# BGU-CS-VIL/DPMMSubClusters.jl

Hardware: AMD Instinct MI355X
Metric: Gibbs iterations/sec, N=10M D=64 NIW (higher is better)
Workload: dtype f32

## Files before the change

### dpmmsubclusters.jl_amd/binding.py

```python
import ctypes
import os
import subprocess

import numpy as np

_HERE = os.path.dirname(os.path.abspath(__file__))
PRIOR_NIW, PRIOR_MULT = 0, 1
MAX_CLUSTERS = 1024

_c_i64p = ctypes.POINTER(ctypes.c_int64)
_c_f32p = ctypes.POINTER(ctypes.c_float)
_c_f64p = ctypes.POINTER(ctypes.c_double)

ABI = [
    ("dpmm_abi_version", ctypes.c_int, []),
    ("dpmm_create", ctypes.c_int, [ctypes.POINTER(ctypes.c_void_p), ctypes.c_int, ctypes.c_int, ctypes.c_int64, ctypes.c_int64, ctypes.c_int, ctypes.c_uint64]),
    ("dpmm_destroy", ctypes.c_int, [ctypes.c_void_p]),
    ("dpmm_last_error", ctypes.c_char_p, [ctypes.c_void_p]),
    ("dpmm_upload_points", ctypes.c_int, [ctypes.c_void_p, _c_f32p, ctypes.c_int64]),
    ("dpmm_upload_points_device", ctypes.c_int, [ctypes.c_void_p, ctypes.c_void_p, ctypes.c_int64]),
    ("dpmm_upload_points_npy", ctypes.c_int, [ctypes.c_void_p, ctypes.c_void_p, ctypes.c_int, ctypes.c_int64, ctypes.c_int]),
    ("dpmm_upload_points_csc", ctypes.c_int, [ctypes.c_void_p, _c_i64p, _c_i64p, _c_f32p, ctypes.c_int]),
    ("dpmm_init_labels", ctypes.c_int, [ctypes.c_void_p, ctypes.c_int, ctypes.c_uint32]),
    ("dpmm_set_labels", ctypes.c_int, [ctypes.c_void_p, _c_i64p, _c_i64p]),
# ... 154 lines not shown
]
SAMPLE_MAX_TRIALS_SPARSE = 4096
SAMPLE_MAX_TRIALS_DENSE = 1 << 24
OPT_SCORE_TABLE_MB = 32
SCORE_MAX_TOP = 16
ABI_MISSING = [
    ("dpmm_score_missing_counts", ctypes.c_int, [ctypes.c_void_p, _c_i64p]),
    ("dpmm_impute_points", ctypes.c_int, [ctypes.c_void_p, _c_f32p, ctypes.c_int64]),
    ("dpmm_impute_points_device", ctypes.c_int, [ctypes.c_void_p, ctypes.c_void_p, ctypes.c_int64]),
]
OPT_SCORE_MISSING = 33
SCORE_MAX_MISSING = 16
_IMPUTE_DRAW_TAIL = [ctypes.c_int64, ctypes.c_int64, ctypes.c_void_p, ctypes.c_uint64, ctypes.c_int64, ctypes.c_int64, ctypes.c_int64]
ABI_IMPUTE = [
    ("dpmm_impute_draw_points", ctypes.c_int, [ctypes.c_void_p, _c_f32p] + _IMPUTE_DRAW_TAIL),
    ("dpmm_impute_draw_points_device", ctypes.c_int, [ctypes.c_void_p, ctypes.c_void_p] + _IMPUTE_DRAW_TAIL),
]
IMPUTE_MAX_DRAWS = 1 << 26

HOST_ALLREDUCE_FN = ctypes.CFUNCTYPE(ctypes.c_int, ctypes.c_void_p, ctypes.c_void_p, ctypes.c_int64, ctypes.c_int)

MASTER_NSCALARS = 8
OPT_SCREEN_MARGIN, OPT_TAIL_SCREEN, OPT_PRESCREEN, OPT_ORDERED_SWEEP, OPT_MULT_FORCE_F32, OPT_STATS_ITEMS, OPT_STATS_GROUPS, OPT_TRACE_SLOW, OPT_LOGLIK_REF_CONST, OPT_WAVE_PRIO, OPT_MULT_NO_U8, OPT_SWEEP_GRID, OPT_SWEEP_QUEUE_ROUNDS, OPT_BALL_SCREEN, OPT_KERNEL_TIMING, OPT_STATS_DERIVE, OPT_NOISE_AHEAD, OPT_REF_BRACKET, OPT_SORT_TILE, OPT_ONE_COLLECTIVE, OPT_BF16_SCREENS, OPT_COMM_TIMEOUT_MS, OPT_DIRECTION_SCREEN, _OPT_RESERVED_24, OPT_MULT_DRAWS_AHEAD, OPT_B3_SUBLABELS, OPT_LEAN_TILES, OPT_MASTER_POLL, OPT_CHAIN_FUSION, OPT_LEAN_DIRECTION, OPT_PAIR_BALL = range(1, 32)


class DpmmError(RuntimeError):
    def __init__(self, code, msg):
        super().__init__(f"libdpmmhip error {code}: {msg}")
        self.code = code


def lib_path():
    return os.path.join(_HERE, "lib", "libdpmmhip.so")


def locked_make(args, lock_dir):
    import fcntl
    os.makedirs(lock_dir, exist_ok=True)
    with open(os.path.join(lock_dir, ".build.lock"), "w") as lk:
        fcntl.flock(lk, fcntl.LOCK_EX)
        try:
            subprocess.check_call(args)
        finally:
            fcntl.flock(lk, fcntl.LOCK_UN)


# ... 772 lines not shown
```

### dpmmsubclusters.jl_amd/csrc/dpmm_api.cpp

```cpp
#include "../../include/dpmm_hip.h"
#include "../../include/dpmm_hip_master.h"
#include "../../include/dpmm_hip_debug.h"
#include "../../include/dpmm_hip_tensor.h"
#include "../../include/dpmm_hip_csc.h"
#include "../../include/dpmm_hip_score.h"
#include "../../include/dpmm_hip_rank.h"
#include "../../include/dpmm_hip_overlap.h"
#include "../../include/dpmm_hip_trace.h"
#include "../../include/dpmm_hip_missing.h"
#include "../../include/dpmm_hip_impute.h"
#include "../../include/dpmm_hip_sample.h"
#include "../../include/dpmm_hip_project.h"

#include <hip/hip_runtime.h>
#include <dlfcn.h>

#include <algorithm>
#include <atomic>
#include <condition_variable>
#include <mutex>
#include <thread>
#include <chrono>
#include <cmath>
#include <cstdio>
// ... 216 lines not shown
    float opt_margin = 50.f;
    int opt_prio = 1;
    int opt_queue_rounds = -1;
    int opt_ball = 1;
    DevBuf<uint32_t> d_sp_frag;
    DevBuf<uint32_t> d_refb_big;
    bool have_refb_big = false;
    DevBuf<uint32_t> d_brk_flag;
    DevBuf<float> d_brk_aref;
    DevBuf<float> d_sp_cons;
    PinBuf<uint32_t> h_need;
    int opt_direction = -1;
    bool sp_ready = false, sp_regime = false;
    unsigned sp_count = 0;
    bool sp_last = false;
    int sp_K = -1;
    int sp_cooldown = 0;
    int opt_b3 = 1;
    bool have_b3 = false;
    int opt_chain = 0x7fffffff & ~(8 | 32);
    int opt_pair_ball = 1;
    bool have_pb = false;
    int opt_lean_dir = 1;
    int opt_master_poll = 1;
    int opt_lean = 1;
    DevBuf<uint32_t> d_hard;
    int hard_flip = 0;
    int perm_nbins = 0;
    PinBuf<uint32_t> h_hard;
    int lean_off = 0;
    bool lean_ran = false;
    int lean_backoff = 15;
    int opt_bf16scr = 1;
    int opt_bracket = 1;
    int opt_timing = 0;
    int opt_tail = 1, opt_prescreen = -1, opt_ordered = 1, opt_force_f32 = 0, opt_trace = 0, opt_ref_const = 0;
    int64_t opt_stats_items = 0;
    int opt_stats_groups = 0;
    void *comm = nullptr;
    int rank = 0, world = 1;
    dpmm_host_allreduce_fn host_fn = nullptr;
    void *host_user = nullptr;
    PinBuf<char> h_red;
    hipEvent_t ev_comm[4] = {nullptr, nullptr, nullptr, nullptr};
    bool have_comm_ev[2] = {false, false};
    int64_t comm_bytes[2] = {0, 0};
// ... 1682 lines not shown
        c->apairs_inflight = false; c->apairs_valid = true;
        c->apairs_req.clear();
    }
    const bool fused_pairs_launched = napairs > 0 && fuse_pairs;
    const bool need_event = !poll || (napairs > 0 && !fuse_pairs);
    if (need_event) HIPCHK(c, hipEventRecord(c->ev_master, c->stream));
    if (napairs > 0 && !fuse_pairs) {
        HIPCHK(c, hipStreamWaitEvent(c->stream2, c->ev_master, 0));
        HIPCHK(c, launch_niw_master_pairs(c->ma, c->d_apairs, napairs, c->d_pairs, c->h_apairs, c->stream2));
        HIPCHK(c, hipEventRecord(c->ev_pairs, c->stream2));
        c->apairs_index.clear();
        for (int p = 0; p < napairs; ++p) c->apairs_index[((uint32_t)c->apairs_req[2 * p] << 16) | (uint32_t)c->apairs_req[2 * p + 1]] = p;
        c->apairs_dirty.assign((size_t)c->master_slots, 0);
        c->apairs_inflight = true; c->apairs_valid = true;
        c->apairs_req.clear();
    }
    if (draw_epoch) {
        const int32_t *hs = c->d_dslots;
        const bool have_normals = normals_by_post || noise_ready(c, draw_epoch, K, c->draw_cur ^ 1);
        if (int rc = noise_join(c)) return rc;
        NiwMasterArgs ma = c->ma;
        ma.mu_draw = c->d_mu_draw[c->draw_cur ^ 1];
        HIPCHK(c, launch_niw_master_draw(ma, hs, K, draw_epoch, c->d_Y[c->draw_cur ^ 1], c->d_ld_sigma[c->draw_cur ^ 1], nullptr, nullptr,
                                         nullptr, nullptr, nullptr, nullptr, c->NB, nullptr, 1 | (have_normals ? 4 : 0), c->stream));
        c->noise_valid = false;
        c->spec_inflight = false; c->spec_valid = true; c->spec_epoch = draw_epoch;
        c->spec_slots.assign(slots, slots + K);
    }
    if (int rc = flush_undo(c)) return rc;
    if (poll) { if (int rc = wait_master_records(c, sm, 3 * (int64_t)K, c->h_apairs, fused_pairs_launched ? napairs : 0)) return rc; }
    else HIPCHK(c, sync_event(c, c->ev_master));
    if (master_marks_left(sm, K)) {
        ++c->dbg_early_wait;
        const auto t0 = std::chrono::steady_clock::now();
        while (master_marks_left(sm, K)) {
            if (std::chrono::steady_clock::now() - t0 > std::chrono::seconds(5)) return fail(c, DPMM_EHIP, "posterior records missing 5 s after the event wait returned");
            HIPCHK(c, sync_stream(c, c->stream));
        }
    }
    c->handover_inflight = false;
    *bad = reinterpret_cast<const uint8_t *>(c->h_out.get());
    *small = sm;
    return DPMM_OK;
}

int dpmm_suffstats_device(dpmm_ctx *c, const int64_t *idx, int n_idx) {
    if (!c) return DPMM_EINVAL;
// ... 40 lines not shown
    if (int rc = noise_flush(c)) return rc;
    if (int rc = ensure_capacity(c, K)) return rc;
    if (int rc = master_capacity(c, 0, K)) return rc;
    if (c->handover_inflight) HIPCHK(c, sync_stream(c, c->stream));
    c->handover_inflight = true;
    float *hlr = reinterpret_cast<float *>(c->h_draw.get()), *hw = hlr + 2 * K;
    memcpy(hlr, lr, sizeof(float) * 2 * K);
    memcpy(hw, w, sizeof(float) * K);
    c->have_tail = c->opt_tail && c->D >= 4 && c->D % 4 == 0 && K > 1;
    const bool ahead = c->spec_valid && c->spec_epoch == epoch && (int)c->spec_slots.size() == K &&
                       memcmp(c->spec_slots.data(), slot_of_cluster, sizeof(int32_t) * K) == 0;
    if (int rc = spec_join(c)) return rc;
    c->spec_valid = false;
    if (int rc = noise_join(c)) return rc;
    if (!ahead) if (int rc = device_list(c, c->d_dslots, c->dslots_shadow, slot_of_cluster, (size_t)K)) return rc;
    const int32_t *hs = c->d_dslots;
    c->draw_cur ^= 1;
    NiwMasterArgs ma = c->ma;
    ma.mu_draw = c->d_mu_draw[c->draw_cur];
    const bool normals = !ahead && noise_ready(c, epoch, K, c->draw_cur);
    c->predictive = false;
    const bool roles = (c->opt_chain & 2) != 0, b3_in_pack = roles && want_b3_images(c), pb_in_pack = b3_in_pack && want_pair_ball(c, K);
    HIPCHK(c, launch_niw_master_draw(ma, hs, K, epoch, c->d_Y[c->draw_cur], c->d_ld_sigma[c->draw_cur], hlr, hw, c->d_Rp, c->d_mup, c->d_cst,
                                     c->have_tail ? c->d_tail : nullptr, c->NB, c->d_work, (ahead ? 2 : (normals ? 7 : 3)) | (roles ? 8 : 0) | (b3_in_pack ? 16 : 0) | (pb_in_pack ? 32 : 0), c->stream));
    if (int rc = direction_tables(c, K, b3_in_pack, pb_in_pack)) return rc;
    c->noise_pending = c->opt_noise_ahead < 0 ? (c->D >= 128 || c->n < 4000000) : c->opt_noise_ahead != 0; c->noise_pend_epoch = epoch + 1; c->noise_pend_nmat = 3 * std::min(K + 4, c->master_K);
    if ((c->opt_chain & 16) && niw_master_can_fuse_pairs(c->ma)) c->noise_pending = false;
    c->work_zeroed = true;
    c->have_screen_prep = false;
    c->K = K;
    c->have_params = true;
    c->predictive = false;
    c->draws_on_device = true;
    return DPMM_OK;
}

int dpmm_niw_master_pairs_ahead(dpmm_ctx *c, const int32_t *slots_i, const int32_t *slots_j, int n) {
    if (!c || n < 0 || (n > 0 && (!slots_i || !slots_j))) return DPMM_EINVAL;
    if (!c->master) return fail(c, DPMM_ESTATE, "dpmm_niw_master_setup first");
    c->apairs_req.clear();
    for (int i = 0; i < n; ++i) {
        if (slots_i[i] < 0 || slots_i[i] >= DPMM_MAX_CLUSTERS || slots_j[i] < 0 || slots_j[i] >= DPMM_MAX_CLUSTERS) { c->apairs_req.clear(); return fail(c, DPMM_EINVAL, "slot out of range"); }
        c->apairs_req.push_back(slots_i[i]); c->apairs_req.push_back(slots_j[i]);
    }
    return DPMM_OK;
}

// ... 499 lines not shown
        case DPMM_OPT_PRESCREEN: c->opt_prescreen = value < 0 ? -1 : (value != 0); return DPMM_OK;
        case DPMM_OPT_ORDERED_SWEEP: c->opt_ordered = value != 0; return DPMM_OK;
        case DPMM_OPT_MULT_FORCE_F32:
            if (c->have_points) return fail(c, DPMM_ESTATE, "DPMM_OPT_MULT_FORCE_F32 must be set before the points are uploaded");
            c->opt_force_f32 = value != 0; return DPMM_OK;
        case DPMM_OPT_STATS_ITEMS:
            if (c->Kcap > 0) return fail(c, DPMM_ESTATE, "DPMM_OPT_STATS_ITEMS must be set before the first parameters / K");
            if (value >= 1) c->chunk_dense = c->chunk = (int)std::max<int64_t>((c->prior == DPMM_PRIOR_NIW && c->D <= 64) ? 32 : 256, ((c->n + (int64_t)value - 1) / (int64_t)value + 3) / 4 * 4);
            if (c->x_sparse) return set_points_chunk(c, true);
            return DPMM_OK;
        case DPMM_OPT_STATS_GROUPS: c->opt_stats_groups = value > 0 ? (int)value : 0; return DPMM_OK;
        case DPMM_OPT_TRACE_SLOW: c->opt_trace = value != 0; return DPMM_OK;
        case DPMM_OPT_LOGLIK_REF_CONST: c->opt_ref_const = value != 0; return DPMM_OK;
        case DPMM_OPT_WAVE_PRIO: c->opt_prio = value != 0; return DPMM_OK;
        case DPMM_OPT_MULT_DRAWS_AHEAD: c->opt_mult_draws_ahead = value != 0; c->mspec_valid = false; return DPMM_OK;
        case DPMM_OPT_SWEEP_QUEUE_ROUNDS: c->opt_queue_rounds = value < 0 ? -1 : (int)value; return DPMM_OK;
        case DPMM_OPT_BALL_SCREEN: c->opt_ball = value != 0; return DPMM_OK;
        case DPMM_OPT_STATS_DERIVE: c->opt_derive = value != 0; c->cache_force = true; return DPMM_OK;
        case DPMM_OPT_NOISE_AHEAD: c->opt_noise_ahead = value < 0 ? -1 : (value != 0); return DPMM_OK;
        case DPMM_OPT_REF_BRACKET: c->opt_bracket = value != 0; return DPMM_OK;
        case DPMM_OPT_COMM_TIMEOUT_MS: c->comm_timeout_ms = value > 0 ? (int)std::min(value, 2.0e9) : 0; return DPMM_OK;
        case DPMM_OPT_BF16_SCREENS: c->opt_bf16scr = value != 0; return DPMM_OK;
        case DPMM_OPT_MASTER_POLL: c->opt_master_poll = value != 0; return DPMM_OK;
        case DPMM_OPT_PAIR_BALL: c->opt_pair_ball = value != 0; if (!c->opt_pair_ball) c->have_pb = false; return DPMM_OK;
        case DPMM_OPT_LEAN_DIRECTION: c->opt_lean_dir = value != 0; c->lean_off = 0; c->lean_backoff = 15; c->lean_ran = false; return DPMM_OK;
        case DPMM_OPT_CHAIN_FUSION: c->opt_chain = value < 0 ? (0x7fffffff & ~(8 | 32)) : (int)value; return DPMM_OK;
        case DPMM_OPT_LEAN_TILES: c->opt_lean = value != 0; c->lean_off = 0; c->lean_backoff = 15; c->lean_ran = false; return DPMM_OK;
        case DPMM_OPT_B3_SUBLABELS: c->opt_b3 = value != 0; if (!c->opt_b3) c->have_b3 = false; return DPMM_OK;
        case DPMM_OPT_DIRECTION_SCREEN:
            c->opt_direction = value < 0 ? -1 : (value != 0);
            if (c->opt_direction == 0) { c->sp_ready = false; c->sp_regime = false; }
            return DPMM_OK;
        case DPMM_OPT_ONE_COLLECTIVE: c->opt_one_collective = value < 0 ? -1 : (value != 0); return DPMM_OK;
        case DPMM_OPT_SORT_TILE: {
            const int t = (int)value;
            if (t != SORT_TILE && t != SORT_TILE_SMALL) return fail(c, DPMM_EINVAL, "DPMM_OPT_SORT_TILE: 512 or 2048");
            if (t < c->sort_tile_min) {
                if (c->n > 16000000) return fail(c, DPMM_ELIMIT, "DPMM_OPT_SORT_TILE: 512-point tiles are limited to shards of 16e6 points");
                HIPCHK(c, hipSetDevice(c->device));
                HIPCHK(c, sync_stream(c, c->stream));
                const int nt = (int)((c->n + t - 1) / t);
                const size_t nbmax = 2 * DPMM_MAX_CLUSTERS;
                DevBuf<int32_t> th, tc, tsp;
                if (th.alloc(sizeof(int32_t) * nbmax * (size_t)std::max(1, nt)) != hipSuccess || tc.alloc(sizeof(int32_t) * nbmax * (size_t)std::max(1, nt)) != hipSuccess ||
                    tsp.alloc(sizeof(int32_t) * (size_t)STEP_SPEC_MAX_BINS * (size_t)std::max(1, nt)) != hipSuccess)
                    return fail(c, DPMM_EHIP, "DPMM_OPT_SORT_TILE: out of device memory for the 512-point tile tables");
// ... 1416 lines not shown
```

### dpmmsubclusters.jl_amd/csrc/niw_master.hip

```cpp
#include <algorithm>
#include "dpmm_device.h"
#include "dpmm_kernels.h"
#include "niw_b3.h"

namespace dpmm {

enum : uint32_t { STREAM_M_NORMAL = 32, STREAM_M_CHI = 33, STREAM_M_XI = 34 };
typedef double f64x4m __attribute__((ext_vector_type(4)));
constexpr int NS = DPMM_MASTER_NSCALARS;

__device__ __forceinline__ double log_mv_gamma_wave(double x, int D, int lane) {
    double t = 0.0;
    for (int d = 1 + lane; d <= D; d += 64) t += lgamma(x + 0.5 * (double)(1 - d));
    for (int o = 32; o > 0; o >>= 1) t += __shfl_xor(t, o);
    return t + (double)D * (double)(D - 1) * 0.25 * 1.1447298858494001741434273513530587;
}

__device__ __forceinline__ double u53(uint32_t a, uint32_t b) {
    return ((double)((((uint64_t)a << 32) | b) >> 11) + 0.5) * (1.0 / 9007199254740992.0);
}
__device__ __forceinline__ double normal_from(const Philox4 &r) {
    const double u1 = u53(r.v[0], r.v[1]), u2 = u53(r.v[2], r.v[3]);
    return sqrt(-2.0 * log(u1)) * cos(6.283185307179586476925 * u2);
}
__device__ __forceinline__ double gamma_mt(double a, uint64_t seed, uint64_t idx, uint32_t epoch) {
    double boost = 1.0;
    if (a < 1.0) {
        const Philox4 ru = philox4x32_10(seed, idx * 64 + 63, epoch, STREAM_M_CHI);
        boost = pow(u53(ru.v[0], ru.v[1]), 1.0 / a);
        a += 1.0;
    }
    const double d = a - 1.0 / 3.0, c = 1.0 / sqrt(9.0 * d);
    for (uint32_t t = 0;; ++t) {
        const double x = normal_from(philox4x32_10(seed, idx * 64 + 2 * t, epoch, STREAM_M_CHI));
        const Philox4 ru = philox4x32_10(seed, idx * 64 + 2 * t + 1, epoch, STREAM_M_CHI);
        const double u = u53(ru.v[0], ru.v[1]);
        double v = 1.0 + c * x;
        if (v <= 0.0) continue;
        v = v * v * v;
        if (u < 1.0 - 0.0331 * x * x * x * x) return (d * v) * boost;
        if (log(u) < 0.5 * x * x + d * (1.0 - v + log(v))) return (d * v) * boost;
        if (t > 60) return (d * v) * boost;
    }
}

__device__ __forceinline__ double bartlett_diag(uint64_t seed, uint64_t id, uint32_t epoch, int r, double nu) {
    return sqrt(2.0 * gamma_mt(0.5 * (nu - (double)r), seed, (id << 16) + (uint64_t)r, epoch));
}

__global__ __launch_bounds__(256) void niw_form_kernel(NiwMasterArgs A, const int32_t *__restrict__ jobs, const double *__restrict__ rows,
                                                       double *__restrict__ small) {
    const int j = blockIdx.x / 3, w = blockIdx.x % 3;
    const int k = jobs[2 * j], s = jobs[2 * j + 1];
    const int D = A.D, DP = A.DP;
    const int64_t stride = A.packed_stride;
    const double *l = rows + (int64_t)(2 * k) * stride, *r = l + stride;
    const double cl = (w != 2) ? 1.0 : 0.0, cr = (w != 1) ? 1.0 : 0.0;
    const int row = 3 * s + w;
    double *P = A.fac + (int64_t)row * DP * DP;
    double *m = A.mean + (int64_t)row * DP;
    __shared__ double sm[DPMM_MASTER_MAXD], sm0[DPMM_MASTER_MAXD];
    const double N = cl * l[0] + cr * r[0];
    const double k0 = A.kappa0, v0 = A.nu0, k1 = k0 + N, v1 = v0 + N;
    if (w == 1 && blockIdx.y == 0) {
        double *dst = A.rows_store + (int64_t)(2 * s) * stride;
        for (int64_t e = threadIdx.x; e < 2 * stride; e += blockDim.x) dst[e] = l[e];
// ... 235 lines not shown
        const double rad = sqrt(-2.0 * log(u1));
        double sn, cs;
        sincos(6.283185307179586476925 * u2, &sn, &cs);
        n0 = rad * cs;
        n1 = (c + 1 < r) ? rad * sn : 0.0;
    }
}
__global__ __launch_bounds__(256) void niw_noise_kernel(NiwMasterArgs A, uint32_t epoch, double *__restrict__ Yall) {
    const int DP = A.DP, HP = DP / 2;
    double *Y = Yall + (int64_t)blockIdx.x * DP * DP;
    for (int p2 = blockIdx.y * 256 + threadIdx.x; p2 < DP * HP; p2 += gridDim.y * 256) {
        const int r = p2 / HP, c = 2 * (p2 - r * HP);
        double n0, n1;
        bartlett_pair(A, (uint64_t)blockIdx.x, epoch, r, c, n0, n1);
        Y[(int64_t)r * DP + c] = n0; Y[(int64_t)r * DP + c + 1] = n1;
    }
}
hipError_t launch_niw_master_noise(const NiwMasterArgs &a, int nmat, uint32_t epoch, double *Y, hipStream_t s) {
    if (nmat <= 0) return hipSuccess;
    DPMM_LAUNCH(niw_noise_kernel, dim3(nmat, a.DP >= 128 ? 8 : (a.DP >= 48 ? 4 : 1)), dim3(256), 0, s, a, epoch, Y);
    return hipGetLastError();
}

__global__ __launch_bounds__(256) void niw_draw_kernel(NiwMasterArgs A, const int32_t *__restrict__ slot_of_cluster, uint32_t epoch,
                                                       double *__restrict__ Yall, float *__restrict__ logdet_sigma, int have_noise) {
    const int k = blockIdx.x / 3, w = blockIdx.x % 3;
    const int row = 3 * slot_of_cluster[k] + w;
    const int D = A.D, DP = A.DP, NB = DP / 16, tid = threadIdx.x;
    const double *L = A.fac + (int64_t)row * DP * DP;
    double *Y = Yall + (int64_t)blockIdx.x * DP * DP;
    const double nu = A.nu[row], kap = A.kap[row];
    const uint64_t id = (uint64_t)blockIdx.x;
#ifdef DPMM_POST_STAMPS
    unsigned long long D0 = __builtin_amdgcn_s_memtime(), Dn = 0, Ds = 0, Dp = 0, Dt = 0, Da = 0, Db = 0;
#define DSTAMP(x) x
#else
#define DSTAMP(x)
#endif
    extern __shared__ double lds[];
    double *T = lds;
    double *Ld = lds + 16 * DP;
    double *xi = Ld + 16 * 17;
    double *Lp = xi + DP;
    if (!have_noise) {
        const int HP = DP / 2;
        for (int p2 = tid; p2 < DP * HP; p2 += 256) {
            const int r = p2 / HP, c = 2 * (p2 - r * HP);
            double n0, n1;
            bartlett_pair(A, id, epoch, r, c, n0, n1);
            Y[(int64_t)r * DP + c] = n0; Y[(int64_t)r * DP + c + 1] = n1;
        }
    }
    __syncthreads();
    for (int r = tid; r < D; r += 256) Y[(int64_t)r * DP + r] = bartlett_diag(A.seed, id, epoch, r, nu);
    for (int d = tid; d < DP; d += 256)
        xi[d] = d < D ? normal_from(philox4x32_10(A.seed, (id << 32) + (uint64_t)d, epoch, STREAM_M_XI)) : 0.0;
    __syncthreads();
    DSTAMP(Dn = __builtin_amdgcn_s_memtime() - D0;)
    { const int a2 = tid >> 4, b2 = tid & 15; const double dv = L[(int64_t)a2 * DP + b2]; Ld[a2 * 17 + b2] = (b2 <= a2) ? dv : 0.0; if (a2 == b2) Ld[a2 * 17 + 16] = 1.0 / dv; }
    __syncthreads();
    for (int ib = 0; ib < NB; ++ib) {
        const int i0 = 16 * ib, ncol = i0 + 16;
        DSTAMP(Da = __builtin_amdgcn_s_memtime();)
        DSTAMP(Db = __builtin_amdgcn_s_memtime(); Ds += Db - Da;)
        {
            const int wave = tid >> 6, li = tid & 15, lg = (tid >> 4) & 3;
            for (int idx = 0; idx <= ib; ++idx) {
                const int turn = idx & 7;
                if ((turn < 4 ? turn : 7 - turn) != wave) continue;
                const int cb = idx;
                const double *yc = Y + (int64_t)lg * DP + 16 * cb + li;
                f64x4m acc = {yc[(int64_t)(i0 + 0) * DP], yc[(int64_t)(i0 + 4) * DP], yc[(int64_t)(i0 + 8) * DP], yc[(int64_t)(i0 + 12) * DP]};
                const double *lp = Lp + lg * 17 + li;
                constexpr int PG = 5;
                const int nch = ib - cb;
                double bA[PG][4], bB[PG][4];
                auto loadg = [&](double (&buf)[PG][4], int ch0) {
#pragma unroll
                    for (int g2 = 0; g2 < PG; ++g2) {
// ... 15 lines not shown
                    loadg(bA, 0);
                    for (int ch0 = 0; ch0 < nch; ch0 += 2 * PG) {
                        if (ch0 + PG < nch) loadg(bB, ch0 + PG);
                        mm(bA, ch0);
                        if (ch0 + 2 * PG < nch) loadg(bA, ch0 + 2 * PG);
                        if (ch0 + PG < nch) mm(bB, ch0 + PG);
                    }
                }
                double *tp = T + lg * DP + 16 * cb + li;
                tp[0] = acc[0]; tp[4 * DP] = acc[1]; tp[8 * DP] = acc[2]; tp[12 * DP] = acc[3];
            }
        }
        __syncthreads();
        DSTAMP(Da = __builtin_amdgcn_s_memtime(); Dp += Da - Db;)
        const int n0 = i0 + 16;
        const bool more = ib + 1 < NB;
        double lnx[16], dnx = 0.0;
        {
            const int kc = (more && tid < n0) ? tid : 0, rb = more ? n0 : 0;
#pragma unroll
            for (int a2 = 0; a2 < 16; ++a2) lnx[a2] = L[(int64_t)(rb + a2) * DP + kc];
            dnx = L[(int64_t)(rb + (tid >> 4)) * DP + rb + (tid & 15)];
        }
        for (int q = tid; q < ncol; q += 256) {
            double t[16];
#pragma unroll
            for (int r = 0; r < 16; ++r) t[r] = T[r * DP + q];
#pragma unroll
            for (int r = 0; r < 16; ++r) {
                const double yv = t[r] * Ld[r * 17 + 16];
                t[r] = yv;
#pragma unroll
                for (int r2 = r + 1; r2 < 16; ++r2) t[r2] = __builtin_fma(-Ld[r2 * 17 + r], yv, t[r2]);
            }
#pragma unroll
            for (int r = 0; r < 16; ++r) Y[(int64_t)(i0 + r) * DP + q] = (q <= i0 + r) ? t[r] : 0.0;
        }
        __syncthreads();
        if (more) {
            if (tid < n0) {
#pragma unroll
                for (int a2 = 0; a2 < 16; ++a2) Lp[tid * 17 + a2] = lnx[a2];
            }
            const int a2 = tid >> 4, b2 = tid & 15;
            Ld[a2 * 17 + b2] = (b2 <= a2) ? dnx : 0.0;
            if (a2 == b2) Ld[a2 * 17 + 16] = 1.0 / dnx;
        }
        __syncthreads();
        DSTAMP(Dt += __builtin_amdgcn_s_memtime() - Da;)
    }
    DSTAMP(Da = __builtin_amdgcn_s_memtime();)
    if (tid < 64) {
        double lg = 0.0;
        for (int d = tid; d < D; d += 64) lg += log(Y[(int64_t)d * DP + d]);
        for (int o = 32; o > 0; o >>= 1) lg += __shfl_xor(lg, o);
        if (tid == 0) logdet_sigma[blockIdx.x] = (float)(-2.0 * lg);
    }
    double *vv = T;
    __syncthreads();
    for (int cb = NB - 1; cb >= 0; --cb) {
        const int c0 = 16 * cb;
        { const int a2 = tid >> 4, b2 = tid & 15; Ld[a2 * 17 + b2] = (b2 <= a2) ? Y[(int64_t)(c0 + a2) * DP + c0 + b2] : 0.0; }
        double yr[16];
        const int rr = tid < c0 ? tid : 0;
#pragma unroll
        for (int a2 = 0; a2 < 16; ++a2) yr[a2] = Y[(int64_t)(c0 + a2) * DP + rr];
        __syncthreads();
        if (tid < 64) {
            const int t16 = tid & 15;
            double xb = xi[c0 + t16];
            const double inv = 1.0 / Ld[t16 * 17 + t16];
            double col[16];
#pragma unroll
            for (int a2 = 0; a2 < 16; ++a2) col[a2] = a2 > t16 ? Ld[a2 * 17 + t16] : 0.0;
            double mine_v = 0.0;
#pragma unroll
            for (int a2 = 15; a2 >= 0; --a2) {
                const double wq = xb * inv;
                const double va = __hiloint2double(__builtin_amdgcn_readlane(__double2hiint(wq), a2), __builtin_amdgcn_readlane(__double2loint(wq), a2));
                mine_v = t16 == a2 ? va : mine_v;
                xb = __builtin_fma(-va, col[a2], xb);
            }
            if (tid < 16) vv[c0 + tid] = mine_v;
        }
        __syncthreads();
        for (int r = tid; r < c0; r += 256) {
            double acc = xi[r];
#pragma unroll
            for (int a2 = 0; a2 < 16; ++a2) acc = __builtin_fma(-vv[c0 + a2], yr[a2], acc);
            xi[r] = acc;
        }
        __syncthreads();
    }
    const double isk = 1.0 / sqrt(kap);
    const double *m = A.mean + (int64_t)row * DP;
    float *mu_out = A.mu_draw + (int64_t)blockIdx.x * DP;
    for (int d = tid; d < DP; d += 256) mu_out[d] = d < D ? (float)(m[d] + vv[d] * isk) : 0.f;
#ifdef DPMM_POST_STAMPS
    __syncthreads();
    if (tid == 0 && blockIdx.x == 3) { float *o = logdet_sigma + 3; o[0] = (float)Dn; o[1] = (float)Ds; o[2] = (float)Dp; o[3] = (float)Dt; o[4] = (float)(__builtin_amdgcn_s_memtime() - Da); o[5] = (float)(__builtin_amdgcn_s_memtime() - D0); }
#endif
}

__global__ __launch_bounds__(256) void niw_draw_inputs_kernel(NiwMasterArgs A, const int32_t *__restrict__ slot_of_cluster, uint32_t epoch,
                                                              double *__restrict__ Aout, double *__restrict__ xiout) {
    const int k = blockIdx.x / 3, w = blockIdx.x % 3;
    const int row = 3 * slot_of_cluster[k] + w;
    const int D = A.D, DP = A.DP, HP = DP / 2, tid = threadIdx.x;
    const double nu = A.nu[row];
    const uint64_t id = (uint64_t)blockIdx.x;
    double *Ao = Aout + (int64_t)blockIdx.x * D * D;
    for (int p2 = tid; p2 < DP * HP; p2 += 256) {
        const int r = p2 / HP, c = 2 * (p2 - r * HP);
        double n0, n1;
        bartlett_pair(A, id, epoch, r, c, n0, n1);
        if (r < D && c < D && c != r) Ao[(int64_t)r * D + c] = n0;
        if (r < D && c + 1 < D && c + 1 != r) Ao[(int64_t)r * D + c + 1] = n1;
    }
    for (int r = tid; r < D; r += 256) Ao[(int64_t)r * D + r] = bartlett_diag(A.seed, id, epoch, r, nu);
    for (int d = tid; d < D; d += 256)
// ... 546 lines not shown
    }
}
hipError_t launch_niw_rows_gather(const double *rows_store, const int32_t *slots, int n, int64_t stride, double *dst, hipStream_t s) {
    const int64_t total = (int64_t)n * 2 * stride;
    const int grid = (int)std::min<int64_t>(4096, (total + 255) / 256);
    DPMM_LAUNCH(niw_rows_gather_kernel, dim3(grid > 0 ? grid : 1), dim3(256), 0, s, rows_store, slots, n, 2 * stride, dst);
    return hipGetLastError();
}

size_t niw_master_lds_bytes(int DP) { return sizeof(double) * ((size_t)34 * DP + 16 * 17 + 256); }

hipError_t launch_niw_master_posterior(const NiwMasterArgs &a, const int32_t *jobs, int njobs, const double *rows, double *small, hipStream_t s) {
    if (njobs <= 0) return hipSuccess;
    if (a.DP <= NIW_POST_LDS_MAXDP) {
        static bool attr_l = false;
        if (!attr_l) { hipFuncSetAttribute((const void *)niw_post_lds_kernel<false>, hipFuncAttributeMaxDynamicSharedMemorySize, (int)niw_post_lds_bytes(NIW_POST_LDS_MAXDP)); attr_l = true; }
        DPMM_LAUNCH(niw_post_lds_kernel<false>, dim3(3 * njobs), dim3(256), niw_post_lds_bytes(a.DP), s, a, jobs, rows, small);
        return hipGetLastError();
    }
    DPMM_LAUNCH(niw_form_kernel, dim3(3 * njobs, a.DP >= 64 ? 16 : 1), dim3(256), 0, s, a, jobs, rows, small);
    static bool attr = false;
    if (!attr) {
        hipFuncSetAttribute((const void *)niw_chol_kernel, hipFuncAttributeMaxDynamicSharedMemorySize, (int)niw_master_lds_bytes(DPMM_MASTER_MAXD));
        hipFuncSetAttribute((const void *)niw_draw_kernel, hipFuncAttributeMaxDynamicSharedMemorySize, (int)niw_master_lds_bytes(DPMM_MASTER_MAXD));
        attr = true;
    }
    DPMM_LAUNCH(niw_chol_kernel, dim3(3 * njobs), dim3(256), niw_master_lds_bytes(a.DP), s, a, jobs, small);
    return hipGetLastError();
}

hipError_t launch_niw_master_draw(const NiwMasterArgs &a, const int32_t *slot_of_cluster, int K, uint32_t epoch, double *Y, float *logdet_sigma,
                                  const float *lr, const float *wts, float *Rp, float *mup, float *cst, float *tail, int NB,
                                  unsigned long long *work, int what, hipStream_t s) {
    static bool attr = false;
    if (!attr) {
        hipFuncSetAttribute((const void *)niw_chol_kernel, hipFuncAttributeMaxDynamicSharedMemorySize, (int)niw_master_lds_bytes(DPMM_MASTER_MAXD));
        hipFuncSetAttribute((const void *)niw_draw_kernel, hipFuncAttributeMaxDynamicSharedMemorySize, (int)niw_master_lds_bytes(DPMM_MASTER_MAXD));
        attr = true;
    }
    if (what & 1) DPMM_LAUNCH(niw_draw_kernel, dim3(3 * K), dim3(256), niw_master_lds_bytes(a.DP), s, a, slot_of_cluster, epoch, Y, logdet_sigma, (what & 4) ? 1 : 0);
    if ((what & 2) && (what & 8)) {
        const int nmat = 3 * K, NP = NB * (NB + 1) / 2, DPs = 16 * NB;
        const bool tl = tail != nullptr && a.D >= 4;
        auto blocks = [](int64_t items, int cap) -> int { return (int)std::max<int64_t>(1, std::min<int64_t>((items + 255) / 256, cap)); };
        PackRoles R;
        R.first[0] = 0;
        R.first[1] = R.first[0] + blocks((int64_t)nmat * NP * 64, 2048);
        R.first[2] = R.first[1] + blocks((int64_t)nmat * (1 + DPs) + (tl ? (int64_t)((K + 1) / 2) * 32 + (int64_t)K * 16 : 0), 512);
        const bool img = tl && NB == 4;
        R.first[3] = R.first[2] + (img ? blocks((int64_t)K * REFB_WORDS, 1024) : 0);
        const bool b3 = img && (what & 16);
        R.first[4] = R.first[3] + (b3 ? blocks((int64_t)2 * K * REFB_WORDS, 2048) : 0);
        R.first[5] = R.first[4] + (b3 ? blocks((int64_t)2 * K * 256, 256) : 0);
        const bool pb = b3 && (what & 32) && K >= 2 && K <= PB_MAXK;
        R.first[6] = R.first[5] + (pb ? K : 0);
        DPMM_LAUNCH(niw_master_pack_roles_kernel, dim3(R.first[6]), dim3(256), 0, s, Y, a.mu_draw, logdet_sigma, lr, wts, Rp, mup, cst, tail, a.D, a.DP, NB,
                    nmat, work, R, b3 ? 1 : 0);
    } else if (what & 2) DPMM_LAUNCH(niw_master_pack_kernel, dim3(512), dim3(256), 0, s, Y, a.mu_draw, logdet_sigma, lr, wts, Rp, mup, cst, tail, a.D, a.DP, NB,
                                     3 * K, work);
    return hipGetLastError();
}

}
// ... 1 lines not shown
```

### include/dpmm_hip.h

```cpp
#ifndef DPMM_HIP_H
#define DPMM_HIP_H

#include <stddef.h>
#include <stdint.h>

#ifdef __cplusplus
extern "C" {
#endif

#define DPMM_ABI_VERSION 3

typedef struct dpmm_ctx dpmm_ctx;

enum { DPMM_PRIOR_NIW = 0, DPMM_PRIOR_MULT = 1 };

enum {
    DPMM_OK = 0,
    DPMM_EINVAL = -1,
    DPMM_ENODEVICE = -2,
    DPMM_EHIP = -3,
    DPMM_ESTATE = -4,
    DPMM_ELIMIT = -5,
    DPMM_ECOMM = -6
};
// ... 7 lines not shown
    DPMM_OPT_STATS_ITEMS = 6,
    DPMM_OPT_STATS_GROUPS = 7,
    DPMM_OPT_TRACE_SLOW = 8,
    DPMM_OPT_LOGLIK_REF_CONST = 9,
    DPMM_OPT_MULT_NO_U8 = 11,
    DPMM_OPT_SWEEP_GRID = 12,
    DPMM_OPT_SWEEP_QUEUE_ROUNDS = 13,
    DPMM_OPT_BALL_SCREEN = 14,
    DPMM_OPT_STATS_DERIVE = 16,
    DPMM_OPT_NOISE_AHEAD = 17,
    DPMM_OPT_REF_BRACKET = 18,
    DPMM_OPT_SORT_TILE = 19,
    DPMM_OPT_COMM_TIMEOUT_MS = 22,
    DPMM_OPT_B3_SUBLABELS = 26,
    DPMM_OPT_LEAN_TILES = 27,
    DPMM_OPT_MASTER_POLL = 28,
    DPMM_OPT_CHAIN_FUSION = 29,
    DPMM_OPT_LEAN_DIRECTION = 30,
    DPMM_OPT_PAIR_BALL = 31,
    DPMM_OPT_MULT_DRAWS_AHEAD = 25,
    DPMM_OPT_DIRECTION_SCREEN = 23,
    DPMM_OPT_BF16_SCREENS = 21,
    DPMM_OPT_ONE_COLLECTIVE = 20,
    DPMM_OPT_KERNEL_TIMING = 15,
    DPMM_OPT_WAVE_PRIO = 10
};

#define DPMM_MAX_CLUSTERS 1024
#define DPMM_MAX_DIM_NIW 256
#define DPMM_MAX_DIM_MULT_SPARSE 65536

int dpmm_abi_version(void);

int dpmm_create(dpmm_ctx **ctx, int prior_kind, int D, int64_t n_local, int64_t first_index,
                int device, uint64_t seed);
int dpmm_destroy(dpmm_ctx *ctx);
const char *dpmm_last_error(const dpmm_ctx *ctx);

int dpmm_upload_points(dpmm_ctx *ctx, const float *X, int64_t ldx);
int dpmm_upload_points_device(dpmm_ctx *ctx, const float *dX, int64_t ldx);
int dpmm_upload_points_npy(dpmm_ctx *ctx, const void *rows, int is_f64, int64_t ld, int nan_to_zero);
int dpmm_upload_points_csc(dpmm_ctx *ctx, const int64_t *colptr, const int64_t *rowval, const float *nzval, int index_base);

int dpmm_init_labels(dpmm_ctx *ctx, int init_clusters, uint32_t epoch);
int dpmm_init_labels_from(dpmm_ctx *ctx, int init_clusters, int first_label, uint32_t epoch);
int dpmm_set_option(dpmm_ctx *ctx, int option, double value);
// ... 65 lines not shown
```

Measured before the change: 706.0.

## Spread NIW posterior draw work across all waves in draw kernel

Adds a templated SPREAD variant of the NIW master draw kernel, on by default behind a new option. Three waves evaluate gamma rejection trials in parallel for the Bartlett diagonal while a fourth draws the normals. The triangular panel solve now has quads of lanes cooperate through shuffles instead of one thread per column. For NB<=4, the mean-draw back-substitution runs in a single wave using readlane broadcasts. The goal is shorter latency in the small per-cluster posterior kernel on the master critical path, at the cost of more code and register pressure.

```diff
diff --git a/dpmmsubclusters.jl_amd/binding.py b/dpmmsubclusters.jl_amd/binding.py
--- a/dpmmsubclusters.jl_amd/binding.py
+++ b/dpmmsubclusters.jl_amd/binding.py
@@ -200,6 +200,7 @@
 
 MASTER_NSCALARS = 8
 OPT_SCREEN_MARGIN, OPT_TAIL_SCREEN, OPT_PRESCREEN, OPT_ORDERED_SWEEP, OPT_MULT_FORCE_F32, OPT_STATS_ITEMS, OPT_STATS_GROUPS, OPT_TRACE_SLOW, OPT_LOGLIK_REF_CONST, OPT_WAVE_PRIO, OPT_MULT_NO_U8, OPT_SWEEP_GRID, OPT_SWEEP_QUEUE_ROUNDS, OPT_BALL_SCREEN, OPT_KERNEL_TIMING, OPT_STATS_DERIVE, OPT_NOISE_AHEAD, OPT_REF_BRACKET, OPT_SORT_TILE, OPT_ONE_COLLECTIVE, OPT_BF16_SCREENS, OPT_COMM_TIMEOUT_MS, OPT_DIRECTION_SCREEN, _OPT_RESERVED_24, OPT_MULT_DRAWS_AHEAD, OPT_B3_SUBLABELS, OPT_LEAN_TILES, OPT_MASTER_POLL, OPT_CHAIN_FUSION, OPT_LEAN_DIRECTION, OPT_PAIR_BALL = range(1, 32)
+OPT_MASTER_PANELS = 34
 
 
 class DpmmError(RuntimeError):
diff --git a/dpmmsubclusters.jl_amd/csrc/dpmm_api.cpp b/dpmmsubclusters.jl_amd/csrc/dpmm_api.cpp
--- a/dpmmsubclusters.jl_amd/csrc/dpmm_api.cpp
+++ b/dpmmsubclusters.jl_amd/csrc/dpmm_api.cpp
@@ -262,6 +262,7 @@
     int opt_pair_ball = 1;
     bool have_pb = false;
     int opt_lean_dir = 1;
+    int opt_master_panels = 1;
     int opt_master_poll = 1;
     int opt_lean = 1;
     DevBuf<uint32_t> d_hard;
@@ -1990,7 +1991,7 @@
         NiwMasterArgs ma = c->ma;
         ma.mu_draw = c->d_mu_draw[c->draw_cur ^ 1];
         HIPCHK(c, launch_niw_master_draw(ma, hs, K, draw_epoch, c->d_Y[c->draw_cur ^ 1], c->d_ld_sigma[c->draw_cur ^ 1], nullptr, nullptr,
-                                         nullptr, nullptr, nullptr, nullptr, c->NB, nullptr, 1 | (have_normals ? 4 : 0), c->stream));
+                                         nullptr, nullptr, nullptr, nullptr, c->NB, nullptr, 1 | (have_normals ? 4 : 0) | (c->opt_master_panels ? 0 : 64), c->stream));
         c->noise_valid = false;
         c->spec_inflight = false; c->spec_valid = true; c->spec_epoch = draw_epoch;
         c->spec_slots.assign(slots, slots + K);
@@ -2077,7 +2078,7 @@
     c->predictive = false;
     const bool roles = (c->opt_chain & 2) != 0, b3_in_pack = roles && want_b3_images(c), pb_in_pack = b3_in_pack && want_pair_ball(c, K);
     HIPCHK(c, launch_niw_master_draw(ma, hs, K, epoch, c->d_Y[c->draw_cur], c->d_ld_sigma[c->draw_cur], hlr, hw, c->d_Rp, c->d_mup, c->d_cst,
-                                     c->have_tail ? c->d_tail : nullptr, c->NB, c->d_work, (ahead ? 2 : (normals ? 7 : 3)) | (roles ? 8 : 0) | (b3_in_pack ? 16 : 0) | (pb_in_pack ? 32 : 0), c->stream));
+                                     c->have_tail ? c->d_tail : nullptr, c->NB, c->d_work, (ahead ? 2 : (normals ? 7 : 3)) | (roles ? 8 : 0) | (b3_in_pack ? 16 : 0) | (pb_in_pack ? 32 : 0) | (c->opt_master_panels ? 0 : 64), c->stream));
     if (int rc = direction_tables(c, K, b3_in_pack, pb_in_pack)) return rc;
     c->noise_pending = c->opt_noise_ahead < 0 ? (c->D >= 128 || c->n < 4000000) : c->opt_noise_ahead != 0; c->noise_pend_epoch = epoch + 1; c->noise_pend_nmat = 3 * std::min(K + 4, c->master_K);
     if ((c->opt_chain & 16) && niw_master_can_fuse_pairs(c->ma)) c->noise_pending = false;
@@ -2623,6 +2624,7 @@
         case DPMM_OPT_COMM_TIMEOUT_MS: c->comm_timeout_ms = value > 0 ? (int)std::min(value, 2.0e9) : 0; return DPMM_OK;
         case DPMM_OPT_BF16_SCREENS: c->opt_bf16scr = value != 0; return DPMM_OK;
         case DPMM_OPT_MASTER_POLL: c->opt_master_poll = value != 0; return DPMM_OK;
+        case DPMM_OPT_MASTER_PANELS: c->opt_master_panels = value != 0; return DPMM_OK;
         case DPMM_OPT_PAIR_BALL: c->opt_pair_ball = value != 0; if (!c->opt_pair_ball) c->have_pb = false; return DPMM_OK;
         case DPMM_OPT_LEAN_DIRECTION: c->opt_lean_dir = value != 0; c->lean_off = 0; c->lean_backoff = 15; c->lean_ran = false; return DPMM_OK;
         case DPMM_OPT_CHAIN_FUSION: c->opt_chain = value < 0 ? (0x7fffffff & ~(8 | 32)) : (int)value; return DPMM_OK;
diff --git a/dpmmsubclusters.jl_amd/csrc/niw_master.hip b/dpmmsubclusters.jl_amd/csrc/niw_master.hip
--- a/dpmmsubclusters.jl_amd/csrc/niw_master.hip
+++ b/dpmmsubclusters.jl_amd/csrc/niw_master.hip
@@ -42,6 +42,28 @@
         if (log(u) < 0.5 * x * x + d * (1.0 - v + log(v))) return (d * v) * boost;
         if (t > 60) return (d * v) * boost;
     }
+}
+
+__device__ __forceinline__ void gamma_mt_prep(double a, uint64_t seed, uint64_t idx, uint32_t epoch, double &boost, double &d, double &c) {
+    boost = 1.0;
+    if (a < 1.0) {
+        const Philox4 ru = philox4x32_10(seed, idx * 64 + 63, epoch, STREAM_M_CHI);
+        boost = pow(u53(ru.v[0], ru.v[1]), 1.0 / a);
+        a += 1.0;
+    }
+    d = a - 1.0 / 3.0; c = 1.0 / sqrt(9.0 * d);
+}
+__device__ __forceinline__ bool gamma_mt_trial(double d, double c, double boost, uint64_t seed, uint64_t idx, uint32_t epoch, uint32_t t, double &out) {
+    const double x = normal_from(philox4x32_10(seed, idx * 64 + 2 * t, epoch, STREAM_M_CHI));
+    const Philox4 ru = philox4x32_10(seed, idx * 64 + 2 * t + 1, epoch, STREAM_M_CHI);
+    const double u = u53(ru.v[0], ru.v[1]);
+    double v = 1.0 + c * x;
+    if (v <= 0.0) return false;
+    v = v * v * v;
+    out = (d * v) * boost;
+    if (u < 1.0 - 0.0331 * x * x * x * x) return true;
+    if (log(u) < 0.5 * x * x + d * (1.0 - v + log(v))) return true;
+    return t > 60;
 }
 
 __device__ __forceinline__ double bartlett_diag(uint64_t seed, uint64_t id, uint32_t epoch, int r, double nu) {
@@ -323,6 +345,7 @@
     return hipGetLastError();
 }
 
+template <bool SPREAD>
 __global__ __launch_bounds__(256) void niw_draw_kernel(NiwMasterArgs A, const int32_t *__restrict__ slot_of_cluster, uint32_t epoch,
                                                        double *__restrict__ Yall, float *__restrict__ logdet_sigma, int have_noise) {
     const int k = blockIdx.x / 3, w = blockIdx.x % 3;
@@ -353,9 +376,36 @@
         }
     }
     __syncthreads();
-    for (int r = tid; r < D; r += 256) Y[(int64_t)r * DP + r] = bartlett_diag(A.seed, id, epoch, r, nu);
-    for (int d = tid; d < DP; d += 256)
-        xi[d] = d < D ? normal_from(philox4x32_10(A.seed, (id << 32) + (uint64_t)d, epoch, STREAM_M_XI)) : 0.0;
+    if (SPREAD && D <= 64) {
+        const int wv = tid >> 6, r = tid & 63;
+        double *gv = T, *gok = T + 3 * DP;
+        if (wv < 3) {
+            if (r < D) {
+                double boost, gd, gc, val = 0.0;
+                gamma_mt_prep(0.5 * (nu - (double)r), A.seed, (id << 16) + (uint64_t)r, epoch, boost, gd, gc);
+                const bool ok = gamma_mt_trial(gd, gc, boost, A.seed, (id << 16) + (uint64_t)r, epoch, (uint32_t)wv, val);
+                gv[wv * DP + r] = val; gok[wv * DP + r] = ok ? 1.0 : 0.0;
+            }
+        } else if (r < DP) xi[r] = r < D ? normal_from(philox4x32_10(A.seed, (id << 32) + (uint64_t)r, epoch, STREAM_M_XI)) : 0.0;
+        __syncthreads();
+        if (tid < D) {
+            double val = 0.0;
+            bool ok = false;
+#pragma unroll
+            for (int t = 0; t < 3; ++t)
+                if (!ok && gok[t * DP + tid] != 0.0) { ok = true; val = gv[t * DP + tid]; }
+            if (!ok) {
+                double boost, gd, gc;
+                gamma_mt_prep(0.5 * (nu - (double)tid), A.seed, (id << 16) + (uint64_t)tid, epoch, boost, gd, gc);
+                for (uint32_t t = 3; !ok; ++t) ok = gamma_mt_trial(gd, gc, boost, A.seed, (id << 16) + (uint64_t)tid, epoch, t, val);
+            }
+            Y[(int64_t)tid * DP + tid] = sqrt(2.0 * val);
+        }
+    } else {
+        for (int r = tid; r < D; r += 256) Y[(int64_t)r * DP + r] = bartlett_diag(A.seed, id, epoch, r, nu);
+        for (int d = tid; d < DP; d += 256)
+            xi[d] = d < D ? normal_from(philox4x32_10(A.seed, (id << 32) + (uint64_t)d, epoch, STREAM_M_XI)) : 0.0;
+    }
     __syncthreads();
     DSTAMP(Dn = __builtin_amdgcn_s_memtime() - D0;)
     { const int a2 = tid >> 4, b2 = tid & 15; const double dv = L[(int64_t)a2 * DP + b2]; Ld[a2 * 17 + b2] = (b2 <= a2) ? dv : 0.0; if (a2 == b2) Ld[a2 * 17 + 16] = 1.0 / dv; }
@@ -417,6 +467,34 @@
             for (int a2 = 0; a2 < 16; ++a2) lnx[a2] = L[(int64_t)(rb + a2) * DP + kc];
             dnx = L[(int64_t)(rb + (tid >> 4)) * DP + rb + (tid & 15)];
         }
+        if constexpr (SPREAD) {
+            const int sq = tid & 3;
+            double cf[16][4], dv[16];
+#pragma unroll
+            for (int r = 0; r < 16; ++r) {
+                dv[r] = Ld[r * 17 + 16];
+#pragma unroll
+                for (int i2 = 0; i2 < 4; ++i2)
+                    if (4 * i2 + 3 > r) cf[r][i2] = Ld[(4 * i2 + sq) * 17 + r];
+            }
+            for (int q = tid >> 2; q < ncol; q += 64) {
+                double wv[4];
+#pragma unroll
+                for (int i2 = 0; i2 < 4; ++i2) wv[i2] = T[(4 * i2 + sq) * DP + q];
+#pragma unroll
+                for (int r = 0; r < 16; ++r) {
+                    const double yv = quad_bcast(wv[r >> 2] * dv[r], r & 3);
+                    if (sq == (r & 3)) wv[r >> 2] = yv;
+#pragma unroll
+                    for (int i2 = 0; i2 < 4; ++i2) {
+                        if (4 * i2 > r) wv[i2] = __builtin_fma(-cf[r][i2], yv, wv[i2]);
+                        else if (4 * i2 + 3 > r) wv[i2] = (4 * i2 + sq > r) ? __builtin_fma(-cf[r][i2], yv, wv[i2]) : wv[i2];
+                    }
+                }
+#pragma unroll
+                for (int i2 = 0; i2 < 4; ++i2) Y[(int64_t)(i0 + 4 * i2 + sq) * DP + q] = (q <= i0 + 4 * i2 + sq) ? wv[i2] : 0.0;
+            }
+        } else
         for (int q = tid; q < ncol; q += 256) {
             double t[16];
 #pragma unroll
@@ -445,11 +523,73 @@
         DSTAMP(Dt += __builtin_amdgcn_s_memtime() - Da;)
     }
     DSTAMP(Da = __builtin_amdgcn_s_memtime();)
+    if (SPREAD && NB <= 4) {
+        const int a2 = tid >> 4, b2 = tid & 15;
+        double dg[4], yr[3][16], lg = 0.0;
+#pragma unroll
+        for (int cb = 0; cb < 4; ++cb) { const int c0 = cb < NB ? 16 * cb : 0; dg[cb] = Y[(int64_t)(c0 + a2) * DP + c0 + b2]; }
+        if (tid < 64) {
+#pragma unroll
+            for (int cb = 1; cb < 4; ++cb) {
+                const int c0 = cb < NB ? 16 * cb : 0, rr = tid < c0 ? tid : 0;
+#pragma unroll
+                for (int r = 0; r < 16; ++r) yr[cb - 1][r] = Y[(int64_t)(c0 + r) * DP + rr];
+            }
+        } else if (tid < 128) {
+            for (int d = tid - 64; d < D; d += 64) lg += log(Y[(int64_t)d * DP + d]);
+            for (int o = 32; o > 0; o >>= 1) lg += __shfl_xor(lg, o);
+#ifdef DPMM_POST_STAMPS
+            if (tid == 64 && !(blockIdx.x > 3 && blockIdx.x < 9)) logdet_sigma[blockIdx.x] = (float)(-2.0 * lg);
+#else
+            if (tid == 64) logdet_sigma[blockIdx.x] = (float)(-2.0 * lg);
+#endif
+        }
+#pragma unroll
+        for (int cb = 0; cb < 4; ++cb)
+            if (cb < NB) Lp[cb * 272 + a2 * 17 + b2] = (b2 <= a2) ? dg[cb] : 0.0;
+        __syncthreads();
+        if (tid < 64) {
+            const int t16 = tid & 15;
+            double xr = tid < DP ? xi[tid] : 0.0, myv = 0.0;
+#pragma unroll
+            for (int cb = 3; cb >= 0; --cb) {
+                if (cb >= NB) continue;
+                const int c0 = 16 * cb;
+                const double *Lb = Lp + cb * 272;
+                double xb = __shfl(xr, c0 + t16);
+                const double inv = 1.0 / Lb[t16 * 17 + t16];
+                double col[16], va[16];
+#pragma unroll
+                for (int r = 0; r < 16; ++r) col[r] = r > t16 ? Lb[r * 17 + t16] : 0.0;
+#pragma unroll
+                for (int r = 15; r >= 0; --r) {
+                    const double wq = xb * inv;
+                    va[r] = __hiloint2double(__builtin_amdgcn_readlane(__double2hiint(wq), r), __builtin_amdgcn_readlane(__double2loint(wq), r));
+                    myv = tid == c0 + r ? va[r] : myv;
+                    xb = __builtin_fma(-va[r], col[r], xb);
+                }
+                if (cb > 0) {
+                    double acc = xr;
+#pragma unroll
+                    for (int r = 0; r < 16; ++r) acc = __builtin_fma(-va[r], yr[cb > 0 ? cb - 1 : 0][r], acc);
+                    xr = tid < c0 ? acc : xr;
+                }
+            }
+            const double isk = 1.0 / sqrt(kap);
+            const double *m = A.mean + (int64_t)row * DP;
+            float *mu_out = A.mu_draw + (int64_t)blockIdx.x * DP;
+            if (tid < DP) mu_out[tid] = tid < D ? (float)(m[tid] + myv * isk) : 0.f;
+        }
+    } else {
     if (tid < 64) {
         double lg = 0.0;
         for (int d = tid; d < D; d += 64) lg += log(Y[(int64_t)d * DP + d]);
         for (int o = 32; o > 0; o >>= 1) lg += __shfl_xor(lg, o);
+#ifdef DPMM_POST_STAMPS
+        if (tid == 0 && !(blockIdx.x > 3 && blockIdx.x < 9)) logdet_sigma[blockIdx.x] = (float)(-2.0 * lg);
+#else
         if (tid == 0) logdet_sigma[blockIdx.x] = (float)(-2.0 * lg);
+#endif
     }
     double *vv = T;
     __syncthreads();
@@ -491,6 +631,7 @@
     const double *m = A.mean + (int64_t)row * DP;
     float *mu_out = A.mu_draw + (int64_t)blockIdx.x * DP;
     for (int d = tid; d < DP; d += 256) mu_out[d] = d < D ? (float)(m[d] + vv[d] * isk) : 0.f;
+    }
 #ifdef DPMM_POST_STAMPS
     __syncthreads();
     if (tid == 0 && blockIdx.x == 3) { float *o = logdet_sigma + 3; o[0] = (float)Dn; o[1] = (float)Ds; o[2] = (float)Dp; o[3] = (float)Dt; o[4] = (float)(__builtin_amdgcn_s_memtime() - Da); o[5] = (float)(__builtin_amdgcn_s_memtime() - D0); }
@@ -1083,7 +1224,8 @@
     static bool attr = false;
     if (!attr) {
         hipFuncSetAttribute((const void *)niw_chol_kernel, hipFuncAttributeMaxDynamicSharedMemorySize, (int)niw_master_lds_bytes(DPMM_MASTER_MAXD));
-        hipFuncSetAttribute((const void *)niw_draw_kernel, hipFuncAttributeMaxDynamicSharedMemorySize, (int)niw_master_lds_bytes(DPMM_MASTER_MAXD));
+        hipFuncSetAttribute((const void *)niw_draw_kernel<true>, hipFuncAttributeMaxDynamicSharedMemorySize, (int)niw_master_lds_bytes(DPMM_MASTER_MAXD));
+        hipFuncSetAttribute((const void *)niw_draw_kernel<false>, hipFuncAttributeMaxDynamicSharedMemorySize, (int)niw_master_lds_bytes(DPMM_MASTER_MAXD));
         attr = true;
     }
     DPMM_LAUNCH(niw_chol_kernel, dim3(3 * njobs), dim3(256), niw_master_lds_bytes(a.DP), s, a, jobs, small);
@@ -1096,10 +1238,12 @@
     static bool attr = false;
     if (!attr) {
         hipFuncSetAttribute((const void *)niw_chol_kernel, hipFuncAttributeMaxDynamicSharedMemorySize, (int)niw_master_lds_bytes(DPMM_MASTER_MAXD));
-        hipFuncSetAttribute((const void *)niw_draw_kernel, hipFuncAttributeMaxDynamicSharedMemorySize, (int)niw_master_lds_bytes(DPMM_MASTER_MAXD));
+        hipFuncSetAttribute((const void *)niw_draw_kernel<true>, hipFuncAttributeMaxDynamicSharedMemorySize, (int)niw_master_lds_bytes(DPMM_MASTER_MAXD));
+        hipFuncSetAttribute((const void *)niw_draw_kernel<false>, hipFuncAttributeMaxDynamicSharedMemorySize, (int)niw_master_lds_bytes(DPMM_MASTER_MAXD));
         attr = true;
     }
-    if (what & 1) DPMM_LAUNCH(niw_draw_kernel, dim3(3 * K), dim3(256), niw_master_lds_bytes(a.DP), s, a, slot_of_cluster, epoch, Y, logdet_sigma, (what & 4) ? 1 : 0);
+    if ((what & 1) && !(what & 64)) DPMM_LAUNCH(niw_draw_kernel<true>, dim3(3 * K), dim3(256), niw_master_lds_bytes(a.DP), s, a, slot_of_cluster, epoch, Y, logdet_sigma, (what & 4) ? 1 : 0);
+    else if (what & 1) DPMM_LAUNCH(niw_draw_kernel<false>, dim3(3 * K), dim3(256), niw_master_lds_bytes(a.DP), s, a, slot_of_cluster, epoch, Y, logdet_sigma, (what & 4) ? 1 : 0);
     if ((what & 2) && (what & 8)) {
         const int nmat = 3 * K, NP = NB * (NB + 1) / 2, DPs = 16 * NB;
         const bool tl = tail != nullptr && a.D >= 4;
diff --git a/include/dpmm_hip.h b/include/dpmm_hip.h
--- a/include/dpmm_hip.h
+++ b/include/dpmm_hip.h
@@ -53,6 +53,7 @@
     DPMM_OPT_DIRECTION_SCREEN = 23,
     DPMM_OPT_BF16_SCREENS = 21,
     DPMM_OPT_ONE_COLLECTIVE = 20,
+    DPMM_OPT_MASTER_PANELS = 34,
     DPMM_OPT_KERNEL_TIMING = 15,
     DPMM_OPT_WAVE_PRIO = 10
 };
```

New measurement: 706.6, median of 2. Within noise of the previous version (+0.1%).
